# Ghoul-tn/DSTAGNN_Drought

Hardware: AMD Instinct MI355X
Metric: DSTAGNN_block fwd+bwd samples/sec (B,N=170,T=12) @1/2/4/8 GPU; %HBM roofline (higher is better)
Workload: dtype fp32; 1 GPU; PEMS08 inner DSTAGNN_block fwd+bwd (train mode, dropout 0.05); global_batch=32, per_gpu_batch=32, N=170, T=12, F=32, K=3, n_heads=3, d_model=512, d_k=32, parallelism=dp1

## Files before the change

dstagnn_drought_amd/csrc/block.hip:

```cpp
#include <algorithm>
#include <atomic>
#include <vector>
#include <cstring>
#include <mutex>
#include <string>

#include "common.hpp"
#include <chrono>
#include <cstdio>
#include <initializer_list>
#include <map>
#include <utility>
#include "ops.hpp"
#include "streams.hpp"

static thread_local std::string g_last_error;
void set_last_error(const std::string& s) { g_last_error = s; }

namespace {

struct Arena {
  char* base;
  size_t off = 0;
  explicit Arena(void* b) : base((char*)b) {}
  float* take(size_t floats) {
    off = (off + 255) & ~size_t(255);
    float* p = base ? (float*)(base + off) : nullptr;
    off += floats * sizeof(float);
    return p;
  }
};

struct Dims {
  int B, N, F, T, h, dk, dv, D, K, C;
  int64_t FT, BFT, BN, NN, HQ, HV, QW, KD, KC, CT, KCT, S;
  int Tg[3], ks[3];
  bool first, sparse, flash;
  bool fsmall;
  bool agg;
  bool tfused;
  int NP;
  bool tfused_bwd;
  bool gfused;
  bool gbfused;
  int64_t tf_wg;
  int64_t nnz;
  int64_t apa_nnz;
};

Dims mkdims(const dstagnn_block_dims& d) {
  Dims m;
  m.B = d.B; m.N = d.N; m.F = d.F; m.T = d.T; m.h = d.n_heads; m.dk = d.d_k; m.dv = d.d_v;
  m.D = d.d_model; m.K = d.K; m.C = d.C;
  m.FT = (int64_t)m.F * m.T; m.BFT = (int64_t)m.B * m.FT; m.BN = (int64_t)m.B * m.N; m.NN = (int64_t)m.N * m.N;
  m.HQ = (int64_t)m.h * m.dk; m.HV = (int64_t)m.h * m.dv; m.QW = 2 * m.HQ + m.HV; m.KD = (int64_t)m.K * m.dk;
  m.KC = (int64_t)m.K * m.C; m.CT = (int64_t)m.C * m.T; m.KCT = m.KC * m.T; m.S = 3 * (int64_t)m.T - 12;
  for (int g = 0; g < 3; ++g) { m.ks[g] = 3 + 2 * g; m.Tg[g] = m.T - m.ks[g] + 1; }
  m.first = (m.F == 1);
  m.sparse = d.cheb_sparse != 0;
  m.flash = m.sparse && d.cheb_flash != 0;
  m.nnz = m.flash ? d.cheb_nnz : 0;
  m.fsmall = m.flash && flash_small(m.N);
  static const bool agg_env = env_flag("DSTAGNN_CHEB_AGG", true);
  m.agg = agg_env && m.sparse && cheb_agg_ok(m.F, m.C, m.K, m.T);
  m.apa_nnz = m.fsmall ? std::max(d.cheb_apa_nnz, 0) : 0;
  m.tfused = tat_fused_fwd_ok(m.N, m.T, m.h, m.dk, m.dv);
  m.NP = m.tfused ? tat_fused_np(m.N) : 0;
  m.tfused_bwd = m.tfused && tat_fused_bwd_ok(m.N, m.T, m.h, m.dk, m.dv, m.F, d.res_mode);
  m.tf_wg = m.tfused_bwd ? tat_fused_bwd_wgs(m.BFT) : 0;
  m.gfused = gtu_fused_fwd_ok(m.C, m.T);
  m.gbfused = gtu_fused_bwd_ok(m.C, m.T);
  return m;
}

struct SaveBufs {
  float *Wqkv, *Wqk, *Wp, *thcat, *Wgf[3], *Wgb[3];
  float* Wqkv_p;
  float *WfcT, *WqT;
  float* Wgt[3];
  float *E, *qkv, *att, *ctx, *u_tat, *mu_tat, *rs_tat, *O, *u_s, *mu_s, *rs_s, *Zd, *qk, *P, *W, *xth, *X;
  float *lse, *psupp, *wsupp;
  float *am, *amt, *papa;
  float* conv[3];
  float *G, *tco, *r, *mu_c, *rs_c, *u_et, *mu_et, *rs_et;
};

SaveBufs plan_save(const Dims& m, Arena& a) {
  SaveBufs s;
  s.Wqkv = a.take(m.QW * m.N);
  s.Wqkv_p = m.tfused ? a.take(m.QW * m.NP) : nullptr;
  s.WfcT = m.tfused_bwd ? a.take(m.HV * m.NP) : nullptr;
  s.WqT = m.tfused_bwd ? a.take(m.QW * m.NP) : nullptr;
  for (int g = 0; g < 3; ++g) s.Wgt[g] = m.gfused ? a.take(2 * (int64_t)m.C * m.C * m.ks[g]) : nullptr;
  s.Wqk = a.take(2 * m.KD * m.D);
  s.Wp = a.take((int64_t)m.D * m.FT);
  s.thcat = a.take((int64_t)m.F * m.KC);
  for (int g = 0; g < 3; ++g) s.Wgf[g] = a.take(2 * (int64_t)m.C * m.C * m.ks[g]);
// ... 7 lines not shown
  s.rs_tat = a.take(m.BFT);
  s.O = a.take(m.BFT * m.N);
  s.u_s = a.take(m.BN * m.D);
  s.mu_s = a.take(m.BN);
  s.rs_s = a.take(m.BN);
  s.Zd = a.take(m.BN * m.D);
  s.qk = a.take(m.BN * 2 * m.KD);
  s.P = m.flash ? nullptr : a.take((int64_t)m.B * m.K * m.NN);
  s.W = m.sparse ? nullptr : a.take((int64_t)m.B * m.K * m.NN);
  s.lse = m.flash ? a.take((int64_t)m.B * m.K * m.N) : nullptr;
  s.psupp = m.flash ? a.take((int64_t)m.B * m.K * m.nnz) : nullptr;
  s.wsupp = m.flash ? a.take((int64_t)m.B * m.K * m.nnz) : nullptr;
  s.am = m.fsmall ? a.take((int64_t)m.K * m.NN) : nullptr;
  s.amt = m.fsmall ? a.take((int64_t)m.K * m.NN) : nullptr;
  s.papa = m.fsmall ? a.take(std::max<int64_t>(1, (int64_t)m.B * m.K * m.apa_nnz)) : nullptr;
  s.xth = a.take(m.BN * m.KCT);
  s.X = a.take(m.BN * m.CT);
  for (int g = 0; g < 3; ++g) s.conv[g] = a.take(m.BN * 2 * m.C * std::max(m.Tg[g], 0));
  s.G = a.take(m.BN * m.C * m.S);
  s.tco = a.take(m.BN * m.CT);
  s.r = a.take(m.BN * m.CT);
  s.mu_c = a.take(m.BN * m.T);
  s.rs_c = a.take(m.BN * m.T);
  if (m.first) {
    s.u_et = a.take((int64_t)m.B * m.T * m.N);
    s.mu_et = a.take((int64_t)m.B * m.T);
    s.rs_et = a.take((int64_t)m.B * m.T);
  } else {
    s.u_et = s.mu_et = s.rs_et = nullptr;
  }
  return s;
}

constexpr size_t kGemmWs = size_t(8) << 20;
constexpr size_t kPart = size_t(2) << 20;

struct Scratch {
  float *gemm_ws, *part;
  float *gemm_ws_side, *part_side, *dWqkv, *dWqk;
  float *dtc, *dX, *gpre, *gcon_t, *bcon_t, *dres_t, *gcon_s, *bcon_s, *gcon_a, *gcon_e, *dconv[3], *dW, *dxth,
      *dthcat, *dqk, *dZd, *dY, *dWp, *dO, *dU, *dE, *dctx, *dqkv, *dscore, *du_et, *dGt;
  float *dzs, *dzs_r, *cc;
};

Scratch plan_scratch(const Dims& m, Arena& a) {
  Scratch s;
  s.gemm_ws = a.take(kGemmWs);
  s.part = a.take(kPart);
  s.dtc = a.take(m.BN * m.CT);
  s.dX = a.take(m.BN * m.CT);
  s.gpre = a.take(m.BN * m.CT);
  s.gemm_ws_side = a.take(kGemmWs);
  s.part_side = a.take(kPart);
  s.dWqkv = a.take(m.QW * m.N);
  s.dWqk = a.take(2 * m.KD * m.D);
  s.gcon_t = a.take(m.gbfused ? std::max<int64_t>(m.BN * m.CT, gtu_fused_bwd_part_floats(m.BN)) : m.BN * m.CT);
  s.bcon_t = a.take(m.BN * m.CT);
  s.dres_t = a.take(m.BN * m.CT);
  s.gcon_s = a.take(m.BN * m.D);
  s.bcon_s = a.take(m.BN * m.D);
  s.gcon_a = a.take(m.BFT * m.N);
  s.gcon_e = m.first ? a.take((int64_t)m.B * m.T * m.N) : nullptr;
  for (int g = 0; g < 3; ++g) s.dconv[g] = a.take((m.BN * m.T + m.ks[g] - 1) * 2 * m.C);
  s.dW = m.flash ? nullptr : a.take((int64_t)m.B * m.K * m.NN);
  s.dzs = m.flash ? a.take((int64_t)m.B * m.K * m.nnz) : nullptr;
  s.dzs_r = m.fsmall ? a.take((int64_t)m.B * m.K * m.nnz) : nullptr;
  s.cc = m.flash ? a.take((int64_t)m.B * m.K * m.N) : nullptr;
  s.dxth = m.agg ? nullptr : a.take(m.BN * m.KCT);
  s.dthcat = a.take((int64_t)m.F * m.KC);
// ... 461 lines not shown
      a.nsrc = 2;
      a.g = p.embS_g; a.b = p.embS_b;
      a.y = s.Zd; a.yrow = idx1(m.D);
      a.u = lean ? nullptr : s.u_s; a.mu = s.mu_s; a.rs = s.rs_s;
      if (d.train && d.drop_p > 0.f) {
        a.drop_p = d.drop_p; a.seed = d.seed; a.which = 0; a.drop_off = drop_off(d, 0);
      }
      DS_TRY(op_ln_fwd(a, st));
    }
    {
      Gemm g;
      g.M = (int)m.BN; g.N = (int)(2 * m.KD); g.K = m.D;
      g.A = s.Zd; g.am = idx1(m.D); g.ak = idx1(1);
      g.B = s.Wqk; g.bk = idx1(1); g.bn = idx1(m.D);
      g.C = s.qk; g.cm = idx1(2 * m.KD); g.cn = idx1(1);
      DS_TRY(run_gemm(g, w.gemm_ws, kGemmWs, st));
    }
    if (!m.flash) {
      Gemm g;
      g.M = m.N; g.N = m.N; g.K = m.dk; g.batch = m.B * m.K;
      g.A = s.qk; g.am = idx1(2 * m.KD); g.ak = idx1(1); g.az = idx2(m.K, m.dk, m.N * 2 * m.KD);
      g.B = s.qk; g.b_off = m.KD; g.bk = idx1(1); g.bn = idx1(2 * m.KD); g.bz = idx2(m.K, m.dk, m.N * 2 * m.KD);
      g.C = s.P; g.cm = idx1(m.N); g.cn = idx1(1); g.cz = idx1(m.NN);
      g.alpha = 1.f / sqrtf((float)m.dk);
      DS_TRY(run_gemm(g, w.gemm_ws, kGemmWs, st));
    }
    return 0;
  }

  ChebIO cheb_io() {
    ChebIO c;
    c.B = m.B; c.N = m.N; c.F = m.F; c.T = m.T; c.K = m.K; c.C = m.C;
    c.x = x; c.S = s.P; c.mask = p.mask; c.g = &gr; c.sparse = m.sparse; c.thcat = s.thcat;
    c.P = s.P; c.W = s.W; c.xth = s.xth; c.X = s.X;
    c.agg = m.agg;
    if (m.flash) {
      fl = make_fl(m, p, gr, s);
      c.fl = &fl;
    }
    return c;
  }
  int stage_cheb() { return cheb_forward(cheb_io(), w.gemm_ws, st); }

  Gemm gtu_conv(int q) {
    const int ks = m.ks[q], Tg = m.Tg[q];
    Gemm g;
    g.M = (int)(m.BN * Tg); g.N = 2 * m.C; g.K = m.C * ks;
    g.A = s.X; g.am = idx2(Tg, m.C, m.CT); g.ak = idx1(1);
    g.B = s.Wgf[q]; g.bk = idx1(2 * m.C); g.bn = idx1(1);
    g.C = s.conv[q]; g.cm = idx1(2 * m.C); g.cn = idx1(1);
    g.bias = p.gtu_b[q];
    return g;
  }

  int stage_tail() {
    if (m.gfused) {
      GtuFusedArgs g;
      g.BN = m.BN; g.C = m.C; g.T = m.T; g.first = m.first;
      g.X = s.X; g.x = x;
      for (int q = 0; q < 3; ++q) { g.wt[q] = s.Wgt[q]; g.bias[q] = p.gtu_b[q]; g.conv[q] = s.conv[q]; }
      g.fcmy_w = p.fcmy_w; g.fcmy_b = p.fcmy_b; g.res_w = p.res_w; g.res_b = p.res_b;
      g.ln_g = p.ln_g; g.ln_b = p.ln_b;
      if (d.train && d.drop_p > 0.f) { g.drop_p = d.drop_p; g.seed = d.seed; g.drop_off = drop_off(d, 1); }
      g.G = s.G; g.tco = s.tco; g.r = s.r; g.mu = s.mu_c; g.rs = s.rs_c; g.out = out;
      return op_gtu_fused_fwd(g, st);
    }
    const Gemm convs[3] = {gtu_conv(0), gtu_conv(1), gtu_conv(2)};
    DS_TRY(run_gemm_group(convs, 3, w.gemm_ws, kGemmWs, st));
    GtuTailArgs t;
    t.BN = m.BN; t.C = m.C; t.T = m.T; t.first = m.first;
    for (int q = 0; q < 3; ++q) t.conv[q] = s.conv[q];
    t.fcmy_w = p.fcmy_w; t.fcmy_b = p.fcmy_b;
    t.X = s.X; t.x = x; t.res_w = p.res_w; t.res_b = p.res_b; t.ln_g = p.ln_g; t.ln_b = p.ln_b;
    if (d.train && d.drop_p > 0.f) { t.drop_p = d.drop_p; t.seed = d.seed; t.drop_off = drop_off(d, 1); }
    t.G = s.G; t.tco = s.tco; t.r = s.r; t.mu = s.mu_c; t.rs = s.rs_c; t.out = out;
    if (lean && gtu_tail_fwd_split(m.C, m.T)) {
      const int64_t per = (int64_t)m.C * m.S, nb = (int64_t)kGemmWs / per;
      if (nb < 1) { set_last_error("gtu_tail: C*(3T-12) exceeds the GEMM workspace"); return DSTAGNN_E_SHAPE; }
      for (int64_t bn0 = 0; bn0 < m.BN; bn0 += nb) {
        GtuTailArgs c = t;
        c.BN = std::min(nb, m.BN - bn0);
        for (int q = 0; q < 3; ++q) c.conv[q] = t.conv[q] + bn0 * m.Tg[q] * 2 * m.C;
        c.X = t.X + bn0 * m.CT;
        c.x = t.x + bn0 * (m.first ? (int64_t)m.T : m.CT);
        c.drop_off = t.drop_off + (uint64_t)(bn0 * m.CT);
        c.out = out + bn0 * m.CT;
        c.tco = c.out;
        c.G = w.gemm_ws;
        DS_TRY(op_gtu_tail_fwd(c, st));
      }
      return 0;
    }
    return op_gtu_tail_fwd(t, st);
  }

  int run() {
    static const bool prof = env_str("DSTAGNN_HOST_PROFILE") != nullptr;
// ... 175 lines not shown
    }
    {
      Gemm dws[3];
      int nw = 0;
      for (int q = 0; q < 3; ++q) {
        const int kw = m.ks[q], Tg = m.Tg[q];
        const int64_t C2 = 2 * (int64_t)m.C;
        const int64_t cs = C2 * m.T;
        if (gd.gtu_w[q]) {
          Gemm& g = dws[nw++];
          g.M = (int)C2; g.N = m.C * kw; g.K = (int)(m.BN * Tg);
          g.A = w.dconv[q]; g.am = idx1(1);
          if (compact) g.ak = idx1(C2);
          else { g.a_off = (kw - 1) * C2; g.ak = idx2(Tg, C2, cs); }
          g.B = s.X; g.bk = idx2(Tg, m.C, m.CT); g.bn = idx1(1);
          g.C = gd.gtu_w[q]; g.cm = idx1((int64_t)m.C * kw); g.cn = idx2(m.C, kw, 1);
          g.ones_out = gd.gtu_b[q];
        } else {
          DS_TRY(colsum_on(ks.side(), w.dconv[q], compact ? m.BN * Tg : m.BN * m.T + kw - 1, (int)C2, 1, gd.gtu_b[q]));
        }
      }
      if (ks.split())
        for (int q = 0; q < nw; ++q) dws[q].splitk_target = kSideSplitK;
      if (nw) DS_TRY(run_gemm_group(dws, nw, ks.split() ? w.gemm_ws_side : w.gemm_ws, kGemmWs, ks.side()));
    }
    return 0;
  }

  int stage_cheb() {
    const int64_t NN = m.NN, KC = m.KC, T = m.T, CT = m.CT, KCT = m.KCT, FT = m.FT;
    const int B = m.B, N = m.N, K = m.K, C = m.C, F = m.F;
    if (m.agg) {
      ChebAg a = make_ag(B, N, K, F, C, m.T, &gr);
      a.x = x; a.thcat = s.thcat; a.P = s.P; a.agg = s.xth; a.g = w.gpre; a.dW = w.dW; a.dx = dx; a.dx_beta = 1.f;
      if (m.flash) {
        a.nnz = (int)m.nnz; a.wsupp = s.wsupp; a.psupp = s.psupp; a.tsupp = gr.tsupp; a.dzs = w.dzs; a.cc = w.cc;
        if (m.fsmall) { a.csc2csr = gr.csc2csr; a.dzs_r = w.dzs_r; }
      }
      DS_TRY(ks.fork_on([&](ForkSig* sig) { return op_cheb_agg_sddmm(a, st, sig); }));
      DS_TRY(op_cheb_agg_spmm_t(a, ks.side()));
      DS_TRY(mark_side(&dx_ready));
      {
        Gemm g;
        g.M = K * F; g.N = C; g.K = B * N * m.T;
        g.A = s.xth; g.am = idx1(T); g.ak = idx2(T, 1, (int64_t)K * FT);
        g.B = w.gpre; g.bk = idx1(C); g.bn = idx1(1);
        bool adjacent = gd.theta[0] != nullptr;
        for (int k = 1; k < K && adjacent; ++k) adjacent = gd.theta[k] == gd.theta[0] + (int64_t)k * F * C;
        if (adjacent) {
          g.C = gd.theta[0]; g.cm = idx1(C); g.cn = idx1(1);
        } else {
          g.C = w.dthcat; g.cm = idx2(F, KC, C); g.cn = idx1(1);
        }
        DS_TRY(sgemm(g));
        if (!adjacent) DS_TRY(unpack_theta(w.dthcat, K, F, C, gd.theta, ks.side()));
      }
    } else if (m.sparse) {
      ChebSp sp = make_sp(B, N, K, C, m.T, &gr);
      sp.P = s.P; sp.xth = s.xth; sp.g = w.gpre; sp.dW = w.dW; sp.dxth = w.dxth;
      if (m.flash) {
        sp.nnz = (int)m.nnz; sp.wsupp = s.wsupp; sp.csr2csc = gr.csr2csc;
        sp.psupp = s.psupp; sp.tsupp = gr.tsupp; sp.dzs = w.dzs; sp.cc = w.cc;
        if (m.fsmall) { sp.csc2csr = gr.csc2csr; sp.dzs_r = w.dzs_r; }
      }
      DS_TRY(fork());
      DS_TRY(op_cheb_spmm_t_bwd(sp, ks.side()));
      DS_TRY(op_cheb_sddmm_bwd(sp, st));
    } else {
      {
        Gemm g;
        g.M = N; g.N = N; g.K = (int)CT; g.batch = B * K;
        g.A = s.xth; g.am = idx1(KCT); g.ak = idx2(C, 1, KC); g.az = idx2(K, C, N * KCT);
        g.B = w.gpre; g.bk = idx1(1); g.bn = idx1(CT); g.bz = idx2(K, 0, N * CT);
        g.C = w.dW; g.cm = idx1(N); g.cn = idx1(1); g.cz = idx1(NN);
        DS_TRY(gemm(g));
      }
      {
        Gemm g;
        g.M = N; g.N = (int)CT; g.K = N; g.batch = B * K;
        g.A = s.W; g.am = idx1(N); g.ak = idx1(1); g.az = idx1(NN);
        g.B = w.gpre; g.bk = idx1(CT); g.bn = idx1(1); g.bz = idx2(K, 0, N * CT);
// ... 585 lines not shown
```

dstagnn_drought_amd/csrc/cheb_agg.hip:

```cpp
#include "common.hpp"
#include "ops.hpp"

namespace {

__device__ __forceinline__ int frow(int r, int h) { return (r & 3) + 8 * (r >> 2) + 4 * h; }

__device__ __forceinline__ void row16(const float* p, bool ok, float (&v)[16]) {
#pragma unroll
  for (int q = 0; q < 4; ++q) {
    const float4 t = ok ? *reinterpret_cast<const float4*>(p + 4 * q) : make_float4(0.f, 0.f, 0.f, 0.f);
    v[4 * q] = t.x; v[4 * q + 1] = t.y; v[4 * q + 2] = t.z; v[4 * q + 3] = t.w;
  }
}

__device__ __forceinline__ int64_t xcd_block(int on) {
  const int64_t p = blockIdx.x;
  if (!on) return p;
  const int64_t per = gridDim.x >> 3;
  return (p & 7) * per + (p >> 3);
}

constexpr int kE = 4;
__device__ __forceinline__ int rl_i(int v, int i) { return __builtin_amdgcn_readlane(v, i); }
__device__ __forceinline__ float rl_f(float v, int i) {
// ... 533 lines not shown
#pragma unroll
          for (int q = 0; q < kNQ; ++q) v[e][q] = vn[e][q];
      }
    }
  }
  floatx16 acc = zero16();
#pragma unroll
  for (int k = 0; k < KM; ++k) {
    if (k >= a.K) break;
    float bt[16];
    row16(a.thcat + (int64_t)min(l32, a.F - 1) * a.KC + k * a.C + 16 * h, l32 < a.F && 16 * h < a.C, bt);
#pragma unroll
    for (int q = 0; q < kNQ; ++q)
      if (lane + 64 * q < nel) hs[lo[q]] = hv[k][q];
    wave_lds_sync();
#pragma unroll
    for (int s = 0; s < 16; ++s) {
      const int c = 16 * h + s;
      const float av = (c < a.C && l32 < Tc) ? hs[l32 * kAs + c] : 0.f;
      acc = __builtin_amdgcn_mfma_f32_32x32x2f32(av, bt[s], acc, 0, 0, 0);
    }
    wave_lds_sync();
  }
  if (l32 >= a.F) return;
  float* dxr = a.dx + ((int64_t)b * a.N + i) * a.F * a.T + (int64_t)l32 * a.T + t0;
#pragma unroll
  for (int r = 0; r < 16; ++r) {
    const int tl = frow(r, h);
    if (tl < Tc) dxr[tl] = a.dx_beta * dxr[tl] + acc[r];
  }
}

template <int kNQ, int KM>
__global__ __launch_bounds__(256) __attribute__((amdgpu_waves_per_eu(gather_wpe<kNQ, 2 * KM>(), 8))) void cheb_agg_spmm_t2_kernel(ChebAg a) {
  static_assert(kNQ <= 8, "T C <= 512");
  __shared__ float Hs[4][32 * kAs];
  const int lane = threadIdx.x & 63, w = threadIdx.x >> 6, h = lane >> 5, l32 = lane & 31;
  const int64_t wv = xcd_block(a.xcd_order) * 4 + w;
  const int npair = (a.B + 1) >> 1;
  if (wv >= (int64_t)npair * a.N) return;
  const int bp = (int)(wv / a.N), i = (int)(wv % a.N), b0 = 2 * bp, nb = min(2, a.B - b0);
  const int T = a.T, TC = T * a.C;
  const int64_t NN = (int64_t)a.N * a.N;
  float* hs = Hs[w];
  int lo[kNQ];
#pragma unroll
  for (int q = 0; q < kNQ; ++q) {
    const int e = min(lane + 64 * q, TC - 1), tl = e / a.C, c = e - tl * a.C;
    lo[q] = tl * kAs + c;
  }
  const int q0 = a.csr_ptr[i], q1 = a.csr_ptr[i + 1];
  const float* gb0 = a.g + (int64_t)b0 * a.N * TC;
  const float* gb1 = a.g + (int64_t)(b0 + nb - 1) * a.N * TC;
  float hv[2][KM][kNQ];
#pragma unroll
  for (int s = 0; s < 2; ++s)
#pragma unroll
    for (int k = 0; k < KM; ++k)
#pragma unroll
      for (int q = 0; q < kNQ; ++q) hv[s][k][q] = 0.f;
  for (int c0 = q0; c0 < q1; c0 += 32) {
    const int nc = min(32, q1 - c0), nv = 2 * nc, pl = c0 + min(lane, nc - 1);
    const int coll = a.csr_col[pl];
    float wl[2][KM];
    {
      const int ci = a.wsupp ? a.csr2csc[pl] : 0;
      const int64_t o = (int64_t)i * a.N + coll;
#pragma unroll
      for (int s = 0; s < 2; ++s)
#pragma unroll
        for (int k = 0; k < KM; ++k) {
          float ww = 0.f;
          if (k < a.K) {
// ... 3 lines not shown
          }
          wl[s][k] = lane < nc ? ww : 0.f;
        }
    }
    auto gather = [&](int e0, float (&dst)[kE][kNQ]) {
#pragma unroll
      for (int e = 0; e < kE; ++e) {
        const int ve = min(e0 + e, nv - 1);
        const float* gr = ((e & 1) ? gb1 : gb0) + (int64_t)rl_i(coll, ve >> 1) * TC;
#pragma unroll
        for (int q = 0; q < kNQ; ++q) dst[e][q] = gr[min(lane + 64 * q, TC - 1)];
      }
    };
    float v[kE][kNQ];
    gather(0, v);
    for (int e0 = 0; e0 < nv; e0 += kE) {
      float vn[kE][kNQ];
      gather(e0 + kE, vn);
#pragma unroll
      for (int k = 0; k < KM; ++k)
#pragma unroll
        for (int e = 0; e < kE; ++e) {
          const float wk = rl_f(wl[e & 1][k], min((e0 + e) >> 1, 31));
          const float wz = e0 + e < nv ? wk : 0.f;
#pragma unroll
          for (int q = 0; q < kNQ; ++q) hv[e & 1][k][q] = fmaf(wz, v[e][q], hv[e & 1][k][q]);
        }
#pragma unroll
      for (int e = 0; e < kE; ++e)
#pragma unroll
        for (int q = 0; q < kNQ; ++q) v[e][q] = vn[e][q];
    }
  }
  floatx16 acc = zero16();
#pragma unroll
  for (int k = 0; k < KM; ++k) {
    if (k >= a.K) break;
    float bt[16];
    row16(a.thcat + (int64_t)min(l32, a.F - 1) * a.KC + k * a.C + 16 * h, l32 < a.F && 16 * h < a.C, bt);
#pragma unroll
    for (int s = 0; s < 2; ++s) {
      if (s >= nb) break;
#pragma unroll
      for (int q = 0; q < kNQ; ++q)
        if (lane + 64 * q < TC) hs[lo[q] + s * T * kAs] = hv[s][k][q];
    }
    wave_lds_sync();
#pragma unroll
    for (int s = 0; s < 16; ++s) {
      const int c = 16 * h + s;
      const float av = (c < a.C && l32 < nb * T) ? hs[l32 * kAs + c] : 0.f;
      acc = __builtin_amdgcn_mfma_f32_32x32x2f32(av, bt[s], acc, 0, 0, 0);
    }
    wave_lds_sync();
  }
  if (l32 >= a.F) return;
#pragma unroll
  for (int r = 0; r < 16; ++r) {
    const int m = frow(r, h), ms = m >= T ? 1 : 0, mt = m - ms * T;
    if (m < nb * T) {
      float* d = a.dx + ((int64_t)(b0 + ms) * a.N + i) * a.F * T + (int64_t)l32 * T + mt;
      *d = a.dx_beta * *d + acc[r];
    }
  }
}

int nq_of(int n) { return n <= 64 ? 1 : n <= 128 ? 2 : n <= 256 ? 4 : n <= 384 ? 6 : n <= 512 ? 8 : n <= 768 ? 12 : 16; }
int km_of(int K) { return K <= 2 ? 2 : K <= 3 ? 3 : K <= 5 ? 5 : 8; }

ChebAg with_order(const ChebAg& a0) {
  ChebAg a = a0;
  a.xcd_order = (int64_t)a.N * a.F * a.T * (int64_t)sizeof(float) <= (int64_t(4) << 20) ? 1 : 0;
  return a;
}

unsigned grid_rows(int64_t waves) { return (unsigned)(cdiv64(cdiv64(waves, 4), 8) * 8); }

struct Launch {
  const ChebAg& a;
  dim3 grid;
  size_t lds;
  hipStream_t st;
};

template <template <int, int> class Fn>
void dispatch(int nq, int km, const Launch& l) {
#define DS_KM(NQ)                                   \
  switch (km) {                                     \
    case 2: Fn<NQ, 2>::run(l); return;              \
    case 3: Fn<NQ, 3>::run(l); return;              \
    case 5: Fn<NQ, 5>::run(l); return;              \
    default: Fn<NQ, 8>::run(l); return;             \
  }
  switch (nq) {
    case 1: DS_KM(1)
    case 2: DS_KM(2)
    case 4: DS_KM(4)
// ... 51 lines not shown
            done2 = true;
          }
        }
        hipLaunchKernelGGL((cheb_agg_sddmm_kernel<NQ, KM, false>), l.grid, dim3(256), l.lds, l.st, l.a);
        return;
      }
    }
    hipLaunchKernelGGL((cheb_agg_sddmm_kernel<NQ, KM>), l.grid, dim3(256), l.lds, l.st, l.a);
  }
};
template <int NQ, int KM>
struct Sddmm2L {
  static void run(const Launch& l) {
    if constexpr (NQ <= 8) {
      if (l.lds > (64u << 10)) {
        static bool done = false;
        if (!done) {
          (void)hipFuncSetAttribute((const void*)cheb_agg_sddmm2_kernel<NQ, KM>,
                                    hipFuncAttributeMaxDynamicSharedMemorySize, 160 << 10);
          done = true;
        }
      }
      hipLaunchKernelGGL((cheb_agg_sddmm2_kernel<NQ, KM>), l.grid, dim3(256), l.lds, l.st, l.a);
    }
  }
};
template <int NQ, int KM>
struct SpmmT2L {
  static void run(const Launch& l) {
    if constexpr (NQ <= 8) hipLaunchKernelGGL((cheb_agg_spmm_t2_kernel<NQ, KM>), l.grid, dim3(256), 0, l.st, l.a);
  }
};
template <int NQ, int KM>
struct SpmmTL {
  static void run(const Launch& l) {
    hipLaunchKernelGGL((cheb_agg_spmm_t_kernel<NQ, KM>), l.grid, dim3(256), 0, l.st, l.a);
  }
};

int check(const ChebAg& a) {
  if (!cheb_agg_ok(a.F, a.C, a.K, a.T)) {
    set_last_error("cheb_agg: F in 1..32, C in {16, 32}, K in 1..8, SDDMM LDS 16*K*F*T <= 160 KB");
    return DSTAGNN_E_SHAPE;
  }
  return 0;
}

size_t sddmm_lds_bytes(int K, int F, int T) { return (size_t)4 * K * F * T * sizeof(float); }

}

bool cheb_agg_ok(int F, int C, int K, int T) {
  return F >= 1 && F <= 32 && (C == 16 || C == 32) && K >= 1 && K <= 8 && T >= 1 &&
         sddmm_lds_bytes(K, F, T) <= (160u << 10);
}

int op_cheb_agg_fwd(const ChebAg& a0, hipStream_t st) {
  DS_TRY(check(a0));
  const ChebAg a = with_order(a0);
  static const bool pair_env = env_flag("DSTAGNN_AGG_PAIR", true);
  const bool save = a.agg != nullptr;
  if (pair_env && a.T <= 16 && a.F * a.T <= 512) {
    const Launch l{a, dim3(grid_rows((int64_t)((a.B + 1) / 2) * a.N)), 0, st};
    if (save) dispatch<Fwd2L>(nq_of(a.F * a.T), km_of(a.K), l);
    else dispatch<Fwd2NsL>(nq_of(a.F * a.T), km_of(a.K), l);
  } else {
    const Launch l{a, dim3(grid_rows((int64_t)a.B * a.N), (unsigned)cdiv64(a.T, 32)), 0, st};
    if (save) dispatch<FwdL>(nq_of(a.F * std::min(32, a.T)), km_of(a.K), l);
    else dispatch<FwdNsL>(nq_of(a.F * std::min(32, a.T)), km_of(a.K), l);
  }
  DS_CHECK_LAUNCH();
  return 0;
}

int op_cheb_agg_sddmm(const ChebAg& a0, hipStream_t st, ForkSig* sig) {
  DS_TRY(check(a0));
  ChebAg a = with_order(a0);
  if (sig) { a.sig = sig->p; a.sig_v = sig->v; }
  const int FT = a.F * a.T;
  static const bool pair_env = env_flag("DSTAGNN_SDDMM_PAIR", true) &&
                               !env_flag("DSTAGNN_SDDMM_NOPF", false);
  const bool pair = pair_env && a.T <= 16 && FT <= 512 && 2 * sddmm_lds_bytes(a.K, a.F, a.T) <= (160u << 10);
  if (pair) {
    dispatch<Sddmm2L>(nq_of(FT), km_of(a.K),
                      Launch{a, dim3(grid_rows((int64_t)((a.B + 1) / 2) * a.N)), 2 * sddmm_lds_bytes(a.K, a.F, a.T), st});
  } else {
    const size_t lds = sddmm_lds_bytes(a.K, a.F, a.T);
    dispatch<SddmmL>(nq_of(std::min(FT, 1024)), km_of(a.K), Launch{a, dim3(grid_rows((int64_t)a.B * a.N)), lds, st});
  }
  DS_CHECK_LAUNCH();
  if (sig) sig->carried = true;
  return 0;
}

int op_cheb_agg_spmm_t(const ChebAg& a0, hipStream_t st) {
  DS_TRY(check(a0));
  const ChebAg a = with_order(a0);
  static const bool pair_env = env_flag("DSTAGNN_AGG_PAIR", true);
  if (pair_env && a.T <= 16 && a.T * a.C <= 512) {
    dispatch<SpmmT2L>(nq_of(a.T * a.C), km_of(a.K), Launch{a, dim3(grid_rows((int64_t)((a.B + 1) / 2) * a.N)), 0, st});
    DS_CHECK_LAUNCH();
    return 0;
  }
  dispatch<SpmmTL>(nq_of(std::min(32, a.T) * a.C), km_of(a.K),
                   Launch{a, dim3(grid_rows((int64_t)a.B * a.N), (unsigned)cdiv64(a.T, 32)), 0, st});
  DS_CHECK_LAUNCH();
  return 0;
}
```

dstagnn_drought_amd/csrc/gtu_fused.hip:

```cpp
#include <mutex>
#include <set>

#include "common.hpp"
#include "handoff.hpp"
#include "ops.hpp"

namespace {

constexpr int kGC = 32, kGT = 12, kGS = 3 * kGT - 12, kGCT = kGC * kGT;
constexpr int kGNB = 22;
constexpr int kGW = 8;
constexpr int kGXS = kGC + 4;
constexpr int kGSP = kGS + 1;
constexpr int kGMT = (kGNB * (kGT - 2) + 15) / 16;
constexpr int kGMTW = (kGMT + 3) / 4;

__device__ __forceinline__ float gf_sigmoid(float x) { return __builtin_amdgcn_rcpf(1.f + __expf(-x)); }
__device__ __forceinline__ float gf_tanh(float x) {
  const float e = __expf(2.f * fminf(fmaxf(x, -15.f), 15.f));
  return 1.f - 2.f * __builtin_amdgcn_rcpf(e + 1.f);
}

template <int KS, int KN, bool SAVE>
__device__ __forceinline__ void gf_gtu(const GtuFusedArgs& a, int q, int s_off, int64_t bn0, int nn, const float* Xs,
// ... 183 lines not shown
      }
      if (SAVE && tv) {
        *reinterpret_cast<float4*>(a.tco + ge0) = make_float4(tco[0], tco[1], tco[2], tco[3]);
        *reinterpret_cast<float4*>(a.r + ge0) = make_float4(rv[v][0], rv[v][1], rv[v][2], rv[v][3]);
      }
    }
    float mean[4], rs[4];
#pragma unroll
    for (int r = 0; r < 4; ++r) sum[r] = row16_sum(rv[0][r] + rv[1][r]);
#pragma unroll
    for (int r = 0; r < 4; ++r) {
      mean[r] = sum[r] * (1.f / kGC);
      const float d0 = rv[0][r] - mean[r], d1 = rv[1][r] - mean[r];
      rs[r] = d0 * d0 + d1 * d1;
    }
#pragma unroll
    for (int r = 0; r < 4; ++r) rs[r] = rsqrtf(row16_sum(rs[r]) * (1.f / kGC) + 1e-5f);
    if (tv) {
#pragma unroll
      for (int v = 0; v < 2; ++v) {
        float o[4];
#pragma unroll
        for (int r = 0; r < 4; ++r) o[r] = (rv[v][r] - mean[r]) * rs[r] * lg[v] + lb[v];
        *reinterpret_cast<float4*>(a.out + bn0 * kGCT + n * kGCT + (16 * v + i) * kGT + t0) =
            make_float4(o[0], o[1], o[2], o[3]);
      }
      if (SAVE && i == 0) {
        *reinterpret_cast<float4*>(a.mu + (bn0 + n) * kGT + t0) = make_float4(mean[0], mean[1], mean[2], mean[3]);
        *reinterpret_cast<float4*>(a.rs + (bn0 + n) * kGT + t0) = make_float4(rs[0], rs[1], rs[2], rs[3]);
      }
    }
  }
  TF_MARK(6);
  if (SAVE) {
    float4* gout = reinterpret_cast<float4*>(a.G + bn0 * kGC * kGS);
    for (int e4 = tid; e4 < nn * kGC * (kGS / 4); e4 += NT) {
      const int nc = e4 / (kGS / 4), s = 4 * (e4 - nc * (kGS / 4));
      const float* g = Gs + nc * kGSP + s;
      gout[e4] = make_float4(g[0], g[1], g[2], g[3]);
    }
  }
  TF_MARK(7);
  TF_PRINT("gtu_fused", 8);
}

bool gf_al16(const void* p) { return (reinterpret_cast<uintptr_t>(p) & 15) == 0; }

size_t gtu_fused_lds() {
  return sizeof(float) * ((size_t)kGNB * kGT * kGXS + (size_t)kGNB * kGC * kGSP + (size_t)kGNB * kGCT);
}


constexpr int kGBS = 2 * kGC + 4;
constexpr int kGBX = kGC + 4;
constexpr int gb_rows(int q) { return (kGNB * (kGT - 2 - 2 * q) + 15) / 16 * 16; }
constexpr int gb_stage(int q) { return (gb_rows(q) + (3 + 2 * q) * kGC) * kGBS; }
constexpr int gb_cmax(int a, int b) { return a > b ? a : b; }
constexpr int kGBStage = gb_cmax(gb_stage(0), gb_cmax(gb_stage(1), gb_stage(2)));

constexpr int kGBTT = kGC * 13;
constexpr int kGBF = kGT * (kGS + 1);
static_assert(kGW * kGBTT <= kGBStage, "dtc transpose buffers live in the staging region");
constexpr int kGBP = 4 * kGC + kGBF;
constexpr int kGBG1 = 16;

size_t gtu_fused_bwd_lds() {
  return sizeof(float) * ((size_t)kGBStage + (size_t)kGNB * kGT * kGBX + 4 * kGW * kGC + (size_t)kGW * kGBF);
// ... 361 lines not shown
  for (int e = tid; e < kGBP; e += NT)
    st_agent(l2 + (int64_t)g1 * kGBP + e,
             sum_rows_agent<kGBG1>(a.part + (int64_t)g1 * kGBG1 * kGBP + e, kGBP, gsz));
  if (!last_arrival(a.cnt + ng, ng, flag + 1)) return;
  for (int e = tid; e < kGBP; e += NT) {
    float* out;
    int o;
    if (e < 4 * kGC) {
      const int q = e / kGC;
      out = q == 0 ? a.gout : (q == 1 ? a.bout : (q == 2 ? a.rwout : a.rbout));
      o = e - q * kGC;
    } else {
      const int f = e - 4 * kGC, t = f / (kGS + 1), sidx = f - t * (kGS + 1);
      out = sidx < kGS ? a.fwout : a.fbout;
      o = sidx < kGS ? t * kGS + sidx : t;
    }
    if (!out) continue;
    out[o] = sum_rows_agent<kGBG1>(l2 + e, kGBP, ng);
  }
}

}

bool gtu_fused_fwd_ok(int C, int T) {
  static const bool on = env_flag("DSTAGNN_GTU_FUSED", true);
  return on && C == kGC && T == kGT;
}

int op_gtu_fused_fwd(const GtuFusedArgs& a, hipStream_t st) {
  if (!gtu_fused_fwd_ok(a.C, a.T) || a.BN <= 0 || a.BN * kGCT >= (1ll << 31)) {
    set_last_error("gtu_fused_fwd: unsupported shape");
    return DSTAGNN_E_SHAPE;
  }
  const int nsave = (a.G != nullptr) + (a.tco != nullptr) + (a.r != nullptr) + (a.mu != nullptr) + (a.rs != nullptr) +
                    (a.conv[0] != nullptr) + (a.conv[1] != nullptr) + (a.conv[2] != nullptr);
  if (nsave != 0 && nsave != 8) {
    set_last_error("gtu_fused_fwd: saved outputs must be all set or all null");
    return DSTAGNN_E_ARG;
  }
  const bool save = nsave == 8;
  bool al = gf_al16(a.X) && gf_al16(a.x) && gf_al16(a.G) && gf_al16(a.tco) && gf_al16(a.r) && gf_al16(a.mu) &&
            gf_al16(a.rs) && gf_al16(a.out) && gf_al16(a.fcmy_b);
  for (int q = 0; q < 3; ++q) al = al && gf_al16(a.conv[q]) && gf_al16(a.wt[q]) && gf_al16(a.bias[q]);
  if (!al) {
    set_last_error("gtu_fused_fwd: operands must be 16-B aligned");
    return DSTAGNN_E_ARG;
  }
  using Kern = void (*)(GtuFusedArgs);
  const Kern k = save ? (a.first ? gtu_fwd_fused_kernel<true, true> : gtu_fwd_fused_kernel<false, true>)
                      : (a.first ? gtu_fwd_fused_kernel<true, false> : gtu_fwd_fused_kernel<false, false>);
  const size_t lds = gtu_fused_lds();
  {
    static std::mutex mu;
    static std::set<Kern> done;
    std::lock_guard<std::mutex> lock(mu);
    if (!done.count(k)) {
      const hipError_t e = hipFuncSetAttribute((const void*)k, hipFuncAttributeMaxDynamicSharedMemorySize, (int)lds);
      if (e != hipSuccess) { set_last_error(std::string("gtu_fused_fwd: ") + hipGetErrorString(e)); return (int)e; }
      done.insert(k);
    }
  }
  const double flops = 2.0 * a.BN * (2.0 * kGC) * kGC * ((kGT - 2) * 3 + (kGT - 4) * 5 + (kGT - 6) * 7);
  const double bytes = 4.0 * a.BN * (kGCT * 6.0 + 2 * kGC * 24.0 + kGC * kGS);
  void* rec = gemm_prof_begin(flops, bytes, st, DSTAGNN_PROF_GTU_FUSED_FWD);
  hipLaunchKernelGGL(k, dim3((unsigned)cdiv64(a.BN, kGNB)), dim3(kGW * 64), lds, st, a);
  DS_CHECK_LAUNCH();
  gemm_prof_end(rec, st);
  return 0;
}

bool gtu_fused_bwd_ok(int C, int T) {
  static const bool on = env_flag("DSTAGNN_GTU_FUSED_BWD", true);
  return on && C == kGC && T == kGT;
// ... 47 lines not shown
```

dstagnn_drought_amd/csrc/ops.hpp:

```cpp
#pragma once
#include "common.hpp"

struct LnSrc {
  const float* p = nullptr;
  Idx2 row;
  int64_t es = 1;
};

struct LnFwd {
  int R = 0, L = 0;
  LnSrc src[3];
  int nsrc = 0;
  const float* g = nullptr;
  const float* b = nullptr;
  float eps = 1e-5f;
  float* y = nullptr; Idx2 yrow; int64_t yes = 1;
  float* u = nullptr;
  float* mu = nullptr; float* rs = nullptr;
  float drop_p = 0.f; uint64_t seed = 0; uint32_t which = 0;
  uint64_t drop_off = 0;
};

struct LnBwd {
  int R = 0, L = 0;
// ... 110 lines not shown
  float* dW = nullptr;
  float* dxth = nullptr;
  int nnz = 0;
  const float* wsupp = nullptr;
  float* dws = nullptr;
  const float* psupp = nullptr;
  const float* tsupp = nullptr;
  float* dzs = nullptr;
  float* cc = nullptr;
  const int* csc2csr = nullptr;
  float* dzs_r = nullptr;
  const int* csr2csc = nullptr;
  int xcd_order = 0;
};
bool cheb_sparse_ok(int CT);

struct ChebAg {
  int B = 0, N = 0, K = 0, F = 0, C = 0, T = 0, KC = 0, nnz = 0;
  const float* x = nullptr;
  const float* thcat = nullptr;
  const int *csc_ptr = nullptr, *csc_row = nullptr, *csr_ptr = nullptr, *csr_col = nullptr, *csr2csc = nullptr;
  const float* cheb = nullptr;
  const float* P = nullptr;
  const float* wsupp = nullptr;
  float* agg = nullptr;
  float* X = nullptr;
  const float* g = nullptr;
  float* dW = nullptr;
  const float* psupp = nullptr; const float* tsupp = nullptr;
  float* dzs = nullptr; float* dzs_r = nullptr; const int* csc2csr = nullptr; float* cc = nullptr;
  float* dx = nullptr; float dx_beta = 1.f;
  int xcd_order = 0;
  uint32_t* sig = nullptr; uint32_t sig_v = 0;
};
bool cheb_agg_ok(int F, int C, int K, int T);
int op_cheb_agg_fwd(const ChebAg& a, hipStream_t st);
int op_cheb_agg_sddmm(const ChebAg& a, hipStream_t st, ForkSig* sig = nullptr);
int op_cheb_agg_spmm_t(const ChebAg& a, hipStream_t st);

struct ChebFl {
  int B = 0, N = 0, K = 0, nnz = 0, nw = 0;
  float scale = 1.f;
  const float* qk = nullptr; int64_t ld = 0; int kd = 0;
  const float* apa = nullptr;
  const float* mask[DSTAGNN_MAX_K] = {};
  const int32_t* bits = nullptr;
  const int32_t* bits_t = nullptr;
  const int *csc_ptr = nullptr, *csc_row = nullptr, *csr_ptr = nullptr, *csr_col = nullptr, *csr2csc = nullptr;
  const int *apa_ptr = nullptr, *apa_row = nullptr;
  const float* tsupp = nullptr;
  float* lse = nullptr;
  float* psupp = nullptr; float* wsupp = nullptr;
  const float* dws = nullptr; float* dzs = nullptr; float* cc = nullptr;
  float* dqk = nullptr;
  float* dmask[DSTAGNN_MAX_K] = {};
  const float* am = nullptr;
  const float* amt = nullptr;
  float* papa = nullptr; int apa_nnz = 0;
  const int* apa_idx = nullptr;
  const int* apa2t = nullptr;
  float* dzs_r = nullptr;
  uint32_t* sig = nullptr; uint32_t sig_v = 0;
};
bool flash_small(int N);
int op_flash_forward(const ChebFl& a, hipStream_t st);
int op_flash_colc(const ChebFl& a, hipStream_t st);
int op_flash_dqk(const ChebFl& a, hipStream_t st, ForkSig* sig = nullptr);
int op_flash_mask_grad(const ChebFl& a, hipStream_t st);
// ... 118 lines not shown
```

Measured before the change: 60170 samples/s.

## Fuse Chebyshev theta gradient into SpMM-transpose kernel and skip saving GTU G

The backward SpMM-transpose kernel now also accumulates the theta weight gradient with MFMA, from x and the graph-aggregated gradient it already holds in LDS. Each workgroup writes a partial sum, and a new fold kernel reduces those partials into the theta gradient. This removes the forward materialization of the aggregated xth tensor and the separate large-K GEMM over it. Separately, the fused GTU forward no longer stores G when the fused GTU backward is in use, saving a write. In exchange there is extra MFMA and LDS work inside the SpMM kernel, a partial-sum scratch buffer, and an added fold launch.

```diff
diff --git a/dstagnn_drought_amd/csrc/block.hip b/dstagnn_drought_amd/csrc/block.hip
--- a/dstagnn_drought_amd/csrc/block.hip
+++ b/dstagnn_drought_amd/csrc/block.hip
@@ -31,6 +31,9 @@
   }
 };
 
+constexpr size_t kGemmWs = size_t(8) << 20;
+constexpr size_t kPart = size_t(2) << 20;
+
 struct Dims {
   int B, N, F, T, h, dk, dv, D, K, C;
   int64_t FT, BFT, BN, NN, HQ, HV, QW, KD, KC, CT, KCT, S;
@@ -38,6 +41,7 @@
   bool first, sparse, flash;
   bool fsmall;
   bool agg;
+  bool dth;
   bool tfused;
   int NP;
   bool tfused_bwd;
@@ -63,6 +67,7 @@
   m.fsmall = m.flash && flash_small(m.N);
   static const bool agg_env = env_flag("DSTAGNN_CHEB_AGG", true);
   m.agg = agg_env && m.sparse && cheb_agg_ok(m.F, m.C, m.K, m.T);
+  m.dth = m.agg && cheb_agg_dtheta_fused(m.B, m.N, m.F, m.C, m.K, m.T, (int64_t)kGemmWs);
   m.apa_nnz = m.fsmall ? std::max(d.cheb_apa_nnz, 0) : 0;
   m.tfused = tat_fused_fwd_ok(m.N, m.T, m.h, m.dk, m.dv);
   m.NP = m.tfused ? tat_fused_np(m.N) : 0;
@@ -136,9 +141,6 @@
   return s;
 }
 
-constexpr size_t kGemmWs = size_t(8) << 20;
-constexpr size_t kPart = size_t(2) << 20;
-
 struct Scratch {
   float *gemm_ws, *part;
   float *gemm_ws_side, *part_side, *dWqkv, *dWqk;
@@ -666,7 +668,7 @@
     ChebIO c;
     c.B = m.B; c.N = m.N; c.F = m.F; c.T = m.T; c.K = m.K; c.C = m.C;
     c.x = x; c.S = s.P; c.mask = p.mask; c.g = &gr; c.sparse = m.sparse; c.thcat = s.thcat;
-    c.P = s.P; c.W = s.W; c.xth = s.xth; c.X = s.X;
+    c.P = s.P; c.W = s.W; c.xth = m.dth ? nullptr : s.xth; c.X = s.X;
     c.agg = m.agg;
     if (m.flash) {
       fl = make_fl(m, p, gr, s);
@@ -696,7 +698,8 @@
       g.fcmy_w = p.fcmy_w; g.fcmy_b = p.fcmy_b; g.res_w = p.res_w; g.res_b = p.res_b;
       g.ln_g = p.ln_g; g.ln_b = p.ln_b;
       if (d.train && d.drop_p > 0.f) { g.drop_p = d.drop_p; g.seed = d.seed; g.drop_off = drop_off(d, 1); }
-      g.G = s.G; g.tco = s.tco; g.r = s.r; g.mu = s.mu_c; g.rs = s.rs_c; g.out = out;
+      g.G = m.gbfused ? nullptr : s.G;
+      g.tco = s.tco; g.r = s.r; g.mu = s.mu_c; g.rs = s.rs_c; g.out = out;
       return op_gtu_fused_fwd(g, st);
     }
     const Gemm convs[3] = {gtu_conv(0), gtu_conv(1), gtu_conv(2)};
@@ -938,21 +941,28 @@
     const int B = m.B, N = m.N, K = m.K, C = m.C, F = m.F;
     if (m.agg) {
       ChebAg a = make_ag(B, N, K, F, C, m.T, &gr);
-      a.x = x; a.thcat = s.thcat; a.P = s.P; a.agg = s.xth; a.g = w.gpre; a.dW = w.dW; a.dx = dx; a.dx_beta = 1.f;
+      a.x = x; a.thcat = s.thcat; a.P = s.P; a.agg = m.dth ? nullptr : s.xth; a.g = w.gpre; a.dW = w.dW; a.dx = dx; a.dx_beta = 1.f;
+      bool adjacent = gd.theta[0] != nullptr;
+      for (int k = 1; k < K && adjacent; ++k) adjacent = gd.theta[k] == gd.theta[0] + (int64_t)k * F * C;
       if (m.flash) {
         a.nnz = (int)m.nnz; a.wsupp = s.wsupp; a.psupp = s.psupp; a.tsupp = gr.tsupp; a.dzs = w.dzs; a.cc = w.cc;
         if (m.fsmall) { a.csc2csr = gr.csc2csr; a.dzs_r = w.dzs_r; }
       }
       DS_TRY(ks.fork_on([&](ForkSig* sig) { return op_cheb_agg_sddmm(a, st, sig); }));
+      if (m.dth) {
+        a.dth_ws = ks.split() ? w.gemm_ws_side : w.gemm_ws;
+        if (adjacent) { a.dth = gd.theta[0]; a.dth_sk = (int64_t)F * C; a.dth_sf = C; }
+        else { a.dth = w.dthcat; a.dth_sk = C; a.dth_sf = KC; }
+      }
       DS_TRY(op_cheb_agg_spmm_t(a, ks.side()));
       DS_TRY(mark_side(&dx_ready));
-      {
+      if (m.dth) {
+        if (!adjacent) DS_TRY(unpack_theta(w.dthcat, K, F, C, gd.theta, ks.side()));
+      } else {
         Gemm g;
         g.M = K * F; g.N = C; g.K = B * N * m.T;
         g.A = s.xth; g.am = idx1(T); g.ak = idx2(T, 1, (int64_t)K * FT);
         g.B = w.gpre; g.bk = idx1(C); g.bn = idx1(1);
-        bool adjacent = gd.theta[0] != nullptr;
-        for (int k = 1; k < K && adjacent; ++k) adjacent = gd.theta[k] == gd.theta[0] + (int64_t)k * F * C;
         if (adjacent) {
           g.C = gd.theta[0]; g.cm = idx1(C); g.cn = idx1(1);
         } else {
diff --git a/dstagnn_drought_amd/csrc/cheb_agg.hip b/dstagnn_drought_amd/csrc/cheb_agg.hip
--- a/dstagnn_drought_amd/csrc/cheb_agg.hip
+++ b/dstagnn_drought_amd/csrc/cheb_agg.hip
@@ -589,13 +589,21 @@
 }
 
 template <int kNQ, int KM>
+constexpr bool dth_x_lds() { return kNQ == 4 && KM == 3; }
+constexpr bool dth_form_ok(int nq, int km) { return km <= 5 && nq >= 2 && nq <= 8 && !(nq == 2 && km != 3); }
+
+template <int kNQ, int KM, bool DTH = false>
 __global__ __launch_bounds__(256) __attribute__((amdgpu_waves_per_eu(gather_wpe<kNQ, 2 * KM>(), 8))) void cheb_agg_spmm_t2_kernel(ChebAg a) {
   static_assert(kNQ <= 8, "T C <= 512");
+  constexpr bool XL = DTH && dth_x_lds<kNQ, KM>();
   __shared__ float Hs[4][32 * kAs];
+  __shared__ float Xs[XL ? 4 : 1][XL ? 32 * kAs : 1];
   const int lane = threadIdx.x & 63, w = threadIdx.x >> 6, h = lane >> 5, l32 = lane & 31;
-  const int64_t wv = xcd_block(a.xcd_order) * 4 + w;
+  const int64_t wv0 = xcd_block(a.xcd_order) * 4 + w;
   const int npair = (a.B + 1) >> 1;
-  if (wv >= (int64_t)npair * a.N) return;
+  const bool active = wv0 < (int64_t)npair * a.N;
+  if (!DTH && !active) return;
+  const int64_t wv = DTH ? min(wv0, (int64_t)npair * a.N - 1) : wv0;
   const int bp = (int)(wv / a.N), i = (int)(wv % a.N), b0 = 2 * bp, nb = min(2, a.B - b0);
   const int T = a.T, TC = T * a.C;
   const int64_t NN = (int64_t)a.N * a.N;
@@ -665,6 +673,19 @@
         for (int q = 0; q < kNQ; ++q) v[e][q] = vn[e][q];
     }
   }
+  float xa[DTH ? 16 : 1];
+  floatx16 E[DTH ? KM : 1];
+  float* xs = Xs[XL ? w : 0];
+  if constexpr (DTH) {
+#pragma unroll
+    for (int s = 0; s < 16; ++s) {
+      const int m = 2 * s + h, ms = m >= T ? 1 : 0, mt = m - ms * T;
+      xa[s] = (l32 < a.F && m < nb * T) ? a.x[((int64_t)(b0 + ms) * a.N + i) * a.F * T + (int64_t)l32 * T + mt] : 0.f;
+      if constexpr (XL) xs[m * kAs + l32] = xa[s];
+    }
+#pragma unroll
+    for (int k = 0; k < KM; ++k) E[k] = zero16();
+  }
   floatx16 acc = zero16();
 #pragma unroll
   for (int k = 0; k < KM; ++k) {
@@ -685,17 +706,75 @@
       const float av = (c < a.C && l32 < nb * T) ? hs[l32 * kAs + c] : 0.f;
       acc = __builtin_amdgcn_mfma_f32_32x32x2f32(av, bt[s], acc, 0, 0, 0);
     }
+    if constexpr (DTH) {
+#pragma unroll
+      for (int s = 0; s < 16; ++s) {
+        if (2 * s >= nb * T) break;
+        const int m = 2 * s + h;
+        const float bv = (m < nb * T && l32 < a.C) ? hs[m * kAs + l32] : 0.f;
+        const float xv = XL ? xs[m * kAs + l32] : xa[s];
+        E[k] = __builtin_amdgcn_mfma_f32_32x32x2f32(xv, bv, E[k], 0, 0, 0);
+      }
+    }
     wave_lds_sync();
   }
-  if (l32 >= a.F) return;
+  if constexpr (!DTH) {
+    if (l32 >= a.F) return;
+  }
 #pragma unroll
   for (int r = 0; r < 16; ++r) {
     const int m = frow(r, h), ms = m >= T ? 1 : 0, mt = m - ms * T;
-    if (m < nb * T) {
+    if (m < nb * T && (!DTH || (active && l32 < a.F))) {
       float* d = a.dx + ((int64_t)(b0 + ms) * a.N + i) * a.F * T + (int64_t)l32 * T + mt;
       *d = a.dx_beta * *d + acc[r];
     }
   }
+  if constexpr (DTH) {
+    const int FC = a.F * a.C, P = a.K * FC;
+    float* part = a.dth_ws + (int64_t)blockIdx.x * P;
+    __syncthreads();
+#pragma unroll
+    for (int k = 0; k < KM; ++k) {
+      if (k >= a.K) break;
+#pragma unroll
+      for (int r = 0; r < 16; ++r) hs[frow(r, h) * kAs + l32] = active ? E[k][r] : 0.f;
+      __syncthreads();
+      for (int e = threadIdx.x; e < FC; e += 256) {
+        const int f = e / a.C, o = f * kAs + (e - f * a.C);
+        part[k * FC + e] = ((Hs[0][o] + Hs[1][o]) + Hs[2][o]) + Hs[3][o];
+      }
+      __syncthreads();
+    }
+  }
+}
+
+__global__ __launch_bounds__(256) void cheb_agg_dtheta_fold_kernel(const float* part, int nrows, int P, int F, int C,
+                                                                    float* out, int64_t sk, int64_t sf) {
+  __shared__ float4 red[256];
+  const int t = threadIdx.x, sub = t >> 4, q = blockIdx.x * 16 + (t & 15), P4 = P >> 2;
+  float4 v = make_float4(0.f, 0.f, 0.f, 0.f);
+  if (q < P4) {
+    const float4* p = reinterpret_cast<const float4*>(part) + q;
+    for (int r0 = sub; r0 < nrows; r0 += 16 * 8) {
+      float4 u[8];
+#pragma unroll
+      for (int j = 0; j < 8; ++j)
+        u[j] = r0 + 16 * j < nrows ? p[(int64_t)(r0 + 16 * j) * P4] : make_float4(0.f, 0.f, 0.f, 0.f);
+#pragma unroll
+      for (int j = 0; j < 8; ++j) { v.x += u[j].x; v.y += u[j].y; v.z += u[j].z; v.w += u[j].w; }
+    }
+  }
+  red[t] = v;
+  __syncthreads();
+  if (sub != 0 || q >= P4) return;
+  float4 tot = red[t];
+  for (int s = 1; s < 16; ++s) {
+    const float4 x = red[16 * s + t];
+    tot.x += x.x; tot.y += x.y; tot.z += x.z; tot.w += x.w;
+  }
+  const int e = 4 * q, FC = F * C, k = e / FC, r = e - k * FC, f = r / C, c = r - f * C;
+  float* o = out + k * sk + f * sf + c;
+  o[0] = tot.x; o[1] = tot.y; o[2] = tot.z; o[3] = tot.w;
 }
 
 int nq_of(int n) { return n <= 64 ? 1 : n <= 128 ? 2 : n <= 256 ? 4 : n <= 384 ? 6 : n <= 512 ? 8 : n <= 768 ? 12 : 16; }
@@ -813,6 +892,12 @@
   }
 };
 template <int NQ, int KM>
+struct SpmmT2DL {
+  static void run(const Launch& l) {
+    if constexpr (dth_form_ok(NQ, KM)) hipLaunchKernelGGL((cheb_agg_spmm_t2_kernel<NQ, KM, true>), l.grid, dim3(256), 0, l.st, l.a);
+  }
+};
+template <int NQ, int KM>
 struct SpmmTL {
   static void run(const Launch& l) {
     hipLaunchKernelGGL((cheb_agg_spmm_t_kernel<NQ, KM>), l.grid, dim3(256), 0, l.st, l.a);
@@ -829,6 +914,17 @@
 
 size_t sddmm_lds_bytes(int K, int F, int T) { return (size_t)4 * K * F * T * sizeof(float); }
 
+}
+
+int64_t cheb_agg_dtheta_ws_floats(int B, int N, int F, int C, int K) {
+  return (int64_t)grid_rows((int64_t)((B + 1) / 2) * N) * K * F * C;
+}
+
+bool cheb_agg_dtheta_fused(int B, int N, int F, int C, int K, int T, int64_t ws_floats) {
+  static const bool pair_env = env_flag("DSTAGNN_AGG_PAIR", true);
+  if (!pair_env || B < 1 || N < 1 || !cheb_agg_ok(F, C, K, T) || T > 16) return false;
+  if (!dth_form_ok(nq_of(T * C), km_of(K))) return false;
+  return cheb_agg_dtheta_ws_floats(B, N, F, C, K) <= ws_floats;
 }
 
 bool cheb_agg_ok(int F, int C, int K, int T) {
@@ -876,8 +972,22 @@
 
 int op_cheb_agg_spmm_t(const ChebAg& a0, hipStream_t st) {
   DS_TRY(check(a0));
-  const ChebAg a = with_order(a0);
+  ChebAg a = with_order(a0);
   static const bool pair_env = env_flag("DSTAGNN_AGG_PAIR", true);
+  if (a.dth) {
+    if (!a.dth_ws || !cheb_agg_dtheta_fused(a.B, a.N, a.F, a.C, a.K, a.T, cheb_agg_dtheta_ws_floats(a.B, a.N, a.F, a.C, a.K))) {
+      set_last_error("cheb_agg_spmm_t: dTheta in the kernel needs the pair path, K <= 5 and its fold scratch");
+      return DSTAGNN_E_ARG;
+    }
+    const unsigned nwg = grid_rows((int64_t)((a.B + 1) / 2) * a.N);
+    dispatch<SpmmT2DL>(nq_of(a.T * a.C), km_of(a.K), Launch{a, dim3(nwg), 0, st});
+    DS_CHECK_LAUNCH();
+    const int P = a.K * a.F * a.C;
+    hipLaunchKernelGGL(cheb_agg_dtheta_fold_kernel, dim3((unsigned)cdiv64(P / 4, 16)), dim3(256), 0, st, a.dth_ws, (int)nwg,
+                       P, a.F, a.C, a.dth, a.dth_sk, a.dth_sf);
+    DS_CHECK_LAUNCH();
+    return 0;
+  }
   if (pair_env && a.T <= 16 && a.T * a.C <= 512) {
     dispatch<SpmmT2L>(nq_of(a.T * a.C), km_of(a.K), Launch{a, dim3(grid_rows((int64_t)((a.B + 1) / 2) * a.N)), 0, st});
     DS_CHECK_LAUNCH();
diff --git a/dstagnn_drought_amd/csrc/gtu_fused.hip b/dstagnn_drought_amd/csrc/gtu_fused.hip
--- a/dstagnn_drought_amd/csrc/gtu_fused.hip
+++ b/dstagnn_drought_amd/csrc/gtu_fused.hip
@@ -239,7 +239,7 @@
     }
   }
   TF_MARK(6);
-  if (SAVE) {
+  if (SAVE && a.G) {
     float4* gout = reinterpret_cast<float4*>(a.G + bn0 * kGC * kGS);
     for (int e4 = tid; e4 < nn * kGC * (kGS / 4); e4 += NT) {
       const int nc = e4 / (kGS / 4), s = 4 * (e4 - nc * (kGS / 4));
@@ -667,13 +667,13 @@
     set_last_error("gtu_fused_fwd: unsupported shape");
     return DSTAGNN_E_SHAPE;
   }
-  const int nsave = (a.G != nullptr) + (a.tco != nullptr) + (a.r != nullptr) + (a.mu != nullptr) + (a.rs != nullptr) +
+  const int nsave = (a.tco != nullptr) + (a.r != nullptr) + (a.mu != nullptr) + (a.rs != nullptr) +
                     (a.conv[0] != nullptr) + (a.conv[1] != nullptr) + (a.conv[2] != nullptr);
-  if (nsave != 0 && nsave != 8) {
-    set_last_error("gtu_fused_fwd: saved outputs must be all set or all null");
+  if ((nsave != 0 && nsave != 7) || (nsave == 0 && a.G)) {
+    set_last_error("gtu_fused_fwd: saved outputs must be all set (G optional) or all null");
     return DSTAGNN_E_ARG;
   }
-  const bool save = nsave == 8;
+  const bool save = nsave == 7;
   bool al = gf_al16(a.X) && gf_al16(a.x) && gf_al16(a.G) && gf_al16(a.tco) && gf_al16(a.r) && gf_al16(a.mu) &&
             gf_al16(a.rs) && gf_al16(a.out) && gf_al16(a.fcmy_b);
   for (int q = 0; q < 3; ++q) al = al && gf_al16(a.conv[q]) && gf_al16(a.wt[q]) && gf_al16(a.bias[q]);
diff --git a/dstagnn_drought_amd/csrc/ops.hpp b/dstagnn_drought_amd/csrc/ops.hpp
--- a/dstagnn_drought_amd/csrc/ops.hpp
+++ b/dstagnn_drought_amd/csrc/ops.hpp
@@ -166,8 +166,12 @@
   float* dx = nullptr; float dx_beta = 1.f;
   int xcd_order = 0;
   uint32_t* sig = nullptr; uint32_t sig_v = 0;
+  float* dth = nullptr; int64_t dth_sk = 0, dth_sf = 0;
+  float* dth_ws = nullptr;
 };
 bool cheb_agg_ok(int F, int C, int K, int T);
+bool cheb_agg_dtheta_fused(int B, int N, int F, int C, int K, int T, int64_t ws_floats);
+int64_t cheb_agg_dtheta_ws_floats(int B, int N, int F, int C, int K);
 int op_cheb_agg_fwd(const ChebAg& a, hipStream_t st);
 int op_cheb_agg_sddmm(const ChebAg& a, hipStream_t st, ForkSig* sig = nullptr);
 int op_cheb_agg_spmm_t(const ChebAg& a, hipStream_t st);
```

New measurement: 61710 samples/s, median of 6. 1.03x the previous value.
